# google-deepmind/mujoco_mpc

Measured on NVIDIA H100. Metric: env-steps/sec, higher is better.
Workload: dtype f32

## Files before the change

mujoco_mpc_b200/csrc/dev_data.cuh:

```cuda
#pragma once
#include <cuda_runtime.h>

#include "dev_model.h"

#ifndef MJPC_NO_COMPACT
#define MJPC_COMPACT 1
#endif
#ifdef MJPC_COMPACT
#define MJPC_ROLL _Pragma("unroll 1")
#define MJPC_HESS_ROLLED 1
#else
#define MJPC_ROLL
#endif

namespace mjpc_dev {

constexpr int kMaxSplinePoints = 64;
#define MJPC_D_ARRAYS(X)                                                                                          \
  X(qpos, M.nq) X(qvel, M.nv) X(ctrl, M.nu) X(qacc, M.nv) X(qacc_warmstart, M.nv) X(mocap_pos, 3 * M.nmocap)      \
  X(mocap_quat, 4 * M.nmocap) X(xpos, 3 * M.nbody) X(xquat, 4 * M.nbody) X(xmat, 9 * M.nbody)                     \
  X(xipos, 3 * M.nbody) X(ximat, 9 * M.nbody) X(xanchor, 3 * M.njnt) X(xaxis, 3 * M.njnt)                         \
  X(geom_xpos, 3 * M.ngeom) X(geom_xmat, 9 * M.ngeom) X(site_xpos, 3 * M.nsite) X(subtree_com, 3 * M.nbody)       \
  X(cinert, 10 * M.nbody) X(crb, 10 * M.nbody) X(cdof, 6 * M.nv) X(cdof_dot, 6 * M.nv) X(cvel, 6 * M.nbody)       \
  X(cacc, 6 * M.nbody) X(cfrc, 6 * M.nbody) X(cfrc_sub, 6 * M.nbody) X(subtree_linvel, 3 * M.nbody)               \
// ... 61 lines not shown
  const float* gkey;
  int xfrc_on;
  int npseudo;
  int warn;
  float time;
  unsigned* sync;
  int sync_slot;
  int sync_mode;
#ifdef MJPC_PHASE_TIMING
  long long tph[8], tlast;
#endif
};
#ifdef MJPC_PHASE_TIMING
#define PHASE(c, i) do { const long long t_ = clock64(); (c).tph[i] += t_ - (c).tlast; (c).tlast = t_; } while (0)
#else
#define PHASE(c, i) do { } while (0)
#endif
template <int V> struct IntC { static constexpr int v = V; };
constexpr int kHdrWords = (int)((sizeof(DevModel) + 15) / 16) * 4;
constexpr int kLayWords = (int)((sizeof(DevLayout) + 15) / 16) * 4;

struct DynSpec {
  static constexpr bool kStatic = false;
  static constexpr int kNV = 0, kNHPair = 0;
  static constexpr int kWide = 1, kTask = 0;
  static __device__ __forceinline__ const DevModel& hdr(const Ctx& c) { return *reinterpret_cast<const DevModel*>(g_smem + c.hdr); }
  static __device__ __forceinline__ const DevModel& model(const Ctx& c) { return hdr(c); }
  template <int ID> static __device__ __forceinline__ float* mf(const Ctx& c) { return g_smem + hdr(c).fo[ID]; }
  template <int ID> static __device__ __forceinline__ int* mi(const Ctx& c) {
    return reinterpret_cast<int*>(g_smem + c.ibase) + hdr(c).io[ID];
  }
  template <int ID> static __device__ __forceinline__ float* df(const Ctx& c) {
    return g_smem + c.dbase + reinterpret_cast<const DevLayout*>(g_smem + c.lay)->off[ID];
  }
};

template <class K, int W = 1, int T = 0>
struct StaticSpec {
  static constexpr bool kStatic = true;
  static constexpr int kWide = W, kTask = T;
  static __host__ __device__ constexpr int w(size_t byte_off, int i = 0) { return K::kModelWords[byte_off / 4 + i]; }
  struct View {
#define X(n) static constexpr int n = w(offsetof(DevModel, n));
    MJPC_M_INTS(X)
#undef X
  };
  static constexpr int kNV = View::nv, kNHPair = View::nhpair;
  static constexpr int kHdr = View::nf + View::ni;
  static constexpr int kData0 = kHdr + kHdrWords + kLayWords;
  static __device__ __forceinline__ const DevModel& hdr(const Ctx&) { return *reinterpret_cast<const DevModel*>(g_smem + kHdr); }
  static __device__ __forceinline__ View model(const Ctx&) { return View{}; }
  template <int ID> static __device__ __forceinline__ float* mf(const Ctx&) {
    return g_smem + IntC<w(offsetof(DevModel, fo), ID)>::v;
  }
  template <int ID> static __device__ __forceinline__ int* mi(const Ctx&) {
    return reinterpret_cast<int*>(g_smem) + IntC<View::nf + w(offsetof(DevModel, io), ID)>::v;
  }
  template <int ID> static __device__ __forceinline__ float* df(const Ctx&) {
    return g_smem + IntC<kData0 + K::kLayoutOff[ID]>::v;
  }
};

#define CM(c) (SP::hdr(c))
#define MF(n) (SP::template mf<F_##n>(c))
#define MI(n) (SP::template mi<I_##n>(c))
#define DF(n) (SP::template df<D_##n>(c))
#define DI(n) (reinterpret_cast<int*>(SP::template df<D_##n>(c)))

enum { WIDE_EXIT = 0, WIDE_HESSIAN = 1 };
struct WideBox { int cmd, ncon, nlim, ndrow, nefc; int task_exit, task_warn; float task_cost; };
// ... 274 lines not shown
  for (int i = N - 1; i >= 0; i--) {
    const float xi = __shfl_sync(kFull, y, i) * inv[i];
    const float lji = A[i * N + li];
    y = (lane == i) ? xi : (lane < i ? y - lji * xi : y);
  }
  if (lane < N) x[lane] = y;
  __syncwarp();
}

template <int NS>
__device__ __noinline__ void warp_chol_factor_solve(float* A, float* inv, float* x, const float* b, int n, int lane) {
#ifdef MJPC_CHOL_ROLLED2
  if constexpr (NS > 0 && NS <= 32) { warp_chol_factor_solve_rolled<NS>(A, inv, x, b, lane); return; }
  if (n == 18) { warp_chol_factor_solve_rolled<18>(A, inv, x, b, lane); return; }
#endif
#ifndef MJPC_CHOL_ROLLED
  if constexpr (NS > 0 && NS <= 32) { warp_chol_factor_solve_reg<NS>(A, x, b, lane); return; }
  if (n == 18) { warp_chol_factor_solve_reg<18>(A, x, b, lane); return; }
  if (n == 2) { warp_chol_factor_solve_reg<2>(A, x, b, lane); return; }
#endif
  warp_chol(A, inv, n, lane);
  warp_chol_solve(x, A, inv, b, n, lane);
}
#endif

}
```

mujoco_mpc_b200/csrc/dev_model.h:

```cpp
#pragma once
#include <cstdint>
#include <cstring>
#include <stdexcept>
#include <string>
#include <vector>

namespace mjpc_dev {

#define MJPC_F_ARRAYS(X)                                                                                         \
  X(body_pos) X(body_quat) X(body_ipos) X(body_iquat) X(body_mass) X(body_inertia) X(body_subtreemass)           \
  X(body_invweight0) X(jnt_pos) X(jnt_axis) X(jnt_range) X(jnt_stiffness) X(jnt_margin) X(jnt_solref)            \
  X(jnt_solimp) X(qpos0) X(qpos_spring) X(dof_damping) X(dof_armature) X(dof_frictionloss) X(dof_solref)         \
  X(dof_solimp) X(dof_invweight0) X(geom_size) X(geom_pos) X(geom_quat) X(geom_friction) X(geom_solmix)          \
  X(geom_solref) X(geom_solimp) X(geom_margin) X(geom_gap) X(geom_rbound) X(site_pos) X(site_quat)               \
  X(actuator_gear) X(actuator_gainprm) X(actuator_biasprm) X(actuator_ctrlrange) X(actuator_forcerange)          \
  X(key_qpos) X(task_weight) X(task_norm_parameter) X(task_parameters) X(task_state) X(wrap_coef) X(tendon_range)     \
  X(tendon_margin) X(tendon_solref) X(tendon_solimp) X(tendon_invweight0)
#define MJPC_I_ARRAYS(X)                                                                                         \
  X(body_parentid) X(body_rootid) X(body_jntnum) X(body_jntadr) X(body_dofnum) X(body_dofadr) X(body_mocapid)    \
  X(jnt_type) X(jnt_qposadr) X(jnt_dofadr) X(jnt_bodyid) X(jnt_limited) X(dof_bodyid) X(dof_jntid)               \
  X(dof_parentid) X(geom_type) X(geom_bodyid) X(geom_condim) X(geom_priority) X(site_bodyid) X(actuator_trnid) X(actuator_trntype)  \
  X(actuator_biastype) X(actuator_ctrllimited) X(actuator_forcelimited) X(pair_geom1) X(pair_geom2)              \
  X(ray_geoms) X(task_dim_norm_residual) X(task_norm) X(task_num_norm_parameter) X(task_trace_objtype)           \
  X(task_trace_objid) X(task_ids) X(tendon_adr) X(tendon_num) X(tendon_limited) X(wrap_dof) X(wrap_qposadr)
// ... 7 lines not shown
#undef X
      F_COUNT
};
enum IntArrayId {
#define X(n) I_##n,
  MJPC_I_ARRAYS(X) MJPC_I_DERIVED(X)
#undef X
      I_COUNT
};

enum { GEOM_PLANE = 0, GEOM_HFIELD, GEOM_SPHERE, GEOM_CAPSULE, GEOM_ELLIPSOID, GEOM_CYLINDER, GEOM_BOX };
enum { JNT_FREE = 0, JNT_BALL, JNT_SLIDE, JNT_HINGE };
enum { OBJ_BODY = 0, OBJ_XBODY, OBJ_GEOM, OBJ_SITE };
enum { CONE_PYRAMIDAL = 0, CONE_ELLIPTIC = 1 };
enum { RESIDUAL_PARTICLE = 0, RESIDUAL_PARTICLE_COPY = 1, RESIDUAL_CARTPOLE = 2, RESIDUAL_QUADRUPED_FLAT = 3,
       RESIDUAL_HUMANOID_STAND = 4, RESIDUAL_HUMANOID_TRACK = 5, RESIDUAL_SHADOW_REORIENT = 6 };

#define MJPC_M_INTS(X)                                                                                           \
  X(nq) X(nv) X(nu) X(nbody) X(njnt) X(ngeom) X(nsite) X(nmocap) X(nkey) X(npair) X(nray) X(nlevel) X(nmpair)    \
  X(ntendon)                                                                                                     \
  X(nfloss) X(nlimit) X(nhpair) X(cone) X(iterations) X(ls_iterations) X(disable_contact) X(disable_eulerdamp)  \
  X(disable_frictionloss) X(disable_limit) X(disable_refsafe) X(disable_warmstart) X(maxcon) X(maxefc)           \
  X(residual_id) X(num_residual) X(num_term) X(num_trace) X(num_parameters) X(task_state_size) X(any_damping)    \
  X(nf) X(ni)

struct DevModel {
#define X(n) int n;
  MJPC_M_INTS(X)
#undef X
  float timestep, impratio, tolerance, ls_tolerance, meaninertia, risk;
  float differentiable;
  float gravity[3];
  int fo[F_COUNT];
  int io[I_COUNT];
};

struct Blob {
  const uint8_t* p;
  size_t n;
  int nent;
  Blob(const void* data, size_t nbytes) : p((const uint8_t*)data), n(nbytes), nent(0) {
    if (!data || nbytes < 16 || std::memcmp(p, "MJPCB200", 8) != 0) throw std::runtime_error("bad model blob magic");
    std::memcpy(&nent, p + 12, 4);
    if ((size_t)16 + 56 * (size_t)nent > nbytes) throw std::runtime_error("truncated model blob");
  }
  bool find(const char* name, int* dt, int* cnt, int64_t* off) const {
    for (int i = 0; i < nent; i++) {
      const uint8_t* e = p + 16 + 56 * (size_t)i;
      if (std::strncmp((const char*)e, name, 40) == 0) {
        std::memcpy(dt, e + 40, 4); std::memcpy(cnt, e + 44, 4); std::memcpy(off, e + 48, 8);
        if ((size_t)*off + (size_t)*cnt * (*dt ? 8 : 4) > n) throw std::runtime_error("blob entry out of range");
        return true;
      }
    }
// ... 73 lines not shown
  }
  level_adr.push_back((int)level_body.size());
  M.nlevel = maxdepth;
  std::vector<int> subend(nb), lastdof(nb, -1), mlo(nb, 0), mhi(nb, 0);
  for (int bb = 0; bb < nb; bb++) {
    int e = bb + 1;
    while (e < nb && depth[e] > depth[bb]) e++;
    subend[bb] = e;
  }
  for (int bb = 1; bb < nb; bb++) {
    lastdof[bb] = dofnum[bb] > 0 ? dofadr[bb] + dofnum[bb] - 1 : lastdof[parent[bb]];
    uint64_t mask = 0;
    for (int d = lastdof[bb]; d >= 0; d = dofpar[d]) mask |= (uint64_t)1 << d;
    mlo[bb] = (int)(uint32_t)(mask & 0xffffffffu); mhi[bb] = (int)(uint32_t)(mask >> 32);
  }
  std::vector<int> mpi, mpj, fl, lj;
  for (int d = 0; d < nv; d++)
    for (int a = d; a >= 0; a = dofpar[a]) { mpi.push_back(d); mpj.push_back(a); }
  if (!M.disable_frictionloss)
    for (int d = 0; d < nv; d++) if (floss[d] > 0) fl.push_back(d);
  if (!M.disable_limit)
    for (int j = 0; j < M.njnt; j++) if (jlim[j] && (jtype[j] == JNT_SLIDE || jtype[j] == JNT_HINGE)) lj.push_back(j);
  M.nmpair = (int)mpi.size(); M.nfloss = (int)fl.size(); M.nlimit = (int)lj.size();
  M.any_damping = 0;
  for (double x : damping) if (x > 0) M.any_damping = 1;
  auto put = [&](int id, const std::vector<int>& v) { M.io[id] = (int)P.i.size(); P.i.insert(P.i.end(), v.begin(), v.end()); };
  put(I_level_adr, level_adr); put(I_level_body, level_body); put(I_body_subtreeend, subend);
  put(I_body_lastdof, lastdof); put(I_body_dofmask_lo, mlo); put(I_body_dofmask_hi, mhi);
  put(I_mpair_i, mpi); put(I_mpair_j, mpj); put(I_floss_dof, fl); put(I_limit_jnt, lj);
  {
    std::vector<uint8_t> pat((size_t)nv * nv, 0);
    for (size_t k = 0; k < mpi.size(); k++) pat[(size_t)mpi[k] * nv + mpj[k]] = 1;
    auto g1 = b.ints("pair_geom1"), g2 = b.ints("pair_geom2"), gb = b.ints("geom_bodyid");
    auto chain = [&](int bb) { uint64_t m = ((uint64_t)(uint32_t)mhi[bb] << 32) | (uint32_t)mlo[bb]; return m; };
    for (size_t k = 0; k < g1.size(); k++) {
      const uint64_t m1 = chain(gb[g1[k]]), m2 = chain(gb[g2[k]]);
      if (!m1 || !m2) continue;
      const uint64_t mm = m1 | m2;
      for (int r = 0; r < nv; r++) if ((mm >> r) & 1) for (int c2 = 0; c2 <= r; c2++) if ((mm >> c2) & 1) pat[(size_t)r * nv + c2] = 1;
    }
    {
      auto tadr = b.ints("tendon_adr"), tnum = b.ints("tendon_num"), wdof = b.ints("wrap_dof");
      for (size_t t = 0; t < tadr.size(); t++) {
        if (tnum[t] > 16) throw std::runtime_error("a tendon wraps more than 16 dofs (compact Jacobian width)");
        for (int a = tadr[t]; a < tadr[t] + tnum[t]; a++)
          for (int c2 = tadr[t]; c2 < tadr[t] + tnum[t]; c2++) {
// ... 36 lines not shown
```

mujoco_mpc_b200/csrc/dev_physics.cuh:

```cuda
#pragma once
#include "dev_data.cuh"

namespace mjpc_dev {



template <class SP>
__device__ __noinline__ void k_kinematics(Ctx& c) {
  auto&& M = SP::model(c);
  const int lane = c.lane;
  float *xpos = DF(xpos), *xquat = DF(xquat), *xmat = DF(xmat), *xipos = DF(xipos), *ximat = DF(ximat);
  float *xanchor = DF(xanchor), *xaxis = DF(xaxis);
  const float* qpos = DF(qpos);
  if (lane < 3) { xpos[lane] = 0; xipos[lane] = 0; }
  if (lane < 4) xquat[lane] = lane == 0 ? 1.f : 0.f;
  if (lane < 9) { float v = (lane % 4 == 0) ? 1.f : 0.f; xmat[lane] = v; ximat[lane] = v; }
  __syncwarp();
  const int *level_adr = MI(level_adr), *level_body = MI(level_body), *parentid = MI(body_parentid),
            *mocapid = MI(body_mocapid), *jntadr = MI(body_jntadr), *jntnum = MI(body_jntnum),
            *jtype = MI(jnt_type), *jqadr = MI(jnt_qposadr);
  const float *bpos = MF(body_pos), *bquat = MF(body_quat), *bipos = MF(body_ipos), *biquat = MF(body_iquat),
              *jpos = MF(jnt_pos), *jaxis = MF(jnt_axis), *qpos0 = MF(qpos0);
  for (int l = 0; l < M.nlevel; l++) {
    const int a = level_adr[l], e = level_adr[l + 1];
// ... 1014 lines not shown
  }
  __syncwarp();
  float* smooth = DF(qfrc_smooth);
  for (int i = lane; i < nv; i += 32) smooth[i] = passive[i] - bias[i] + qact[i];
  if (c.xfrc_on) {
    const float *xf = DF(xfrc), *cdof = DF(cdof), *xipos = DF(xipos), *scom = DF(subtree_com);
    const int *dbody = MI(dof_bodyid), *subend = MI(body_subtreeend), *rootid = MI(body_rootid);
    for (int i = lane; i < nv; i += 32) {
      const int b0 = dbody[i];
      const float* cd = cdof + 6 * i;
      float a = 0.f;
      MJPC_ROLL
      for (int b = b0; b < subend[b0]; b++) {
        float off[3], t[3];
        for (int q = 0; q < 3; q++) off[q] = xipos[3 * b + q] - scom[3 * rootid[b] + q];
        cross3(t, cd, off);
        const float* f = xf + 6 * b;
        for (int q = 0; q < 3; q++) a += (cd[3 + q] + t[q]) * f[q] + cd[q] * f[3 + q];
      }
      smooth[i] += a;
    }
  }
  __syncwarp();
  warp_chol_factor_solve<SP::kNV>(DF(qLD), DF(ldinv), DF(qacc_smooth), smooth, nv, lane);
}

template <class SP>
__device__ __noinline__ void k_reference(Ctx& c) {
  const int lane = c.lane;
  const float *qvel = DF(qvel), *K = DF(efc_K), *B = DF(efc_B), *imp = DF(efc_imp), *pos = DF(efc_pos),
              *margin = DF(efc_margin);
  float* aref = DF(efc_aref);
  const int nsimple = SP::model(c).nfloss + c.nlim;
  for (int i = lane; i < c.nefc; i += 32) {
    const float v = row_dot<SP>(c, i, nsimple, qvel);
    aref[i] = -B[i] * v - K[i] * imp[i] * (pos[i] - margin[i]);
  }
  __syncwarp();
}

template <class SP>
__device__ __noinline__ float k_update_constraint(Ctx& c, bool hess) {
  auto&& M = SP::model(c);
  const int lane = c.lane, nv = M.nv;
  const float *jar = DF(efc_jar), *D = DF(efc_D), *R = DF(efc_R), *floss = DF(efc_floss), *J = DF(efc_J);
  float *force = DF(efc_force), *X = DF(efc_W), *hw = DF(efc_hw), *xw = DF(efc_hc);
  int *state = DI(efc_state);
// ... 768 lines not shown
      const int i = min(b0 + lane, nv - 1);
      const bool on = b0 + lane < nv;
      const float a = Ma[i] - smooth[i] - qfc[i];
      if (on) grad[i] = a;
      g2 += on ? a * a : 0.f;
      const float m = fabsf(Ma[i]) + fabsf(smooth[i]) + fabsf(qfc[i]);
      ga += on ? m * m : 0.f;
    }
    const float gnorm2 = warp_sum(g2), gabs2 = warp_sum(ga);
    __syncwarp();
    if (iter > 0) {
      const float improvement = (old - cost) / scale_inv, gradient = sqrtf(gnorm2) / scale_inv;
      const float gfloor = kGradFloor * 1.1920929e-7f * sqrtf(gabs2) / scale_inv;
      if (gradient < fmaxf(tol, gfloor)) break;
      const bool resolvable = fabsf(old - cost) > 16.f * 1.1920929e-7f * fabsf(cost);
      if (resolvable) { if (improvement < tol) break; stalls = 0; }
      else if (gradient > 0.5f * prev_gradient && (alpha > 0.5f || ++stalls >= 3)) break;
      prev_gradient = gradient;
    }
    if (iter == M.iterations) break;
    PHASE(c, 4);
    k_hessian<SP>(c);
    PHASE(c, 5);
    warp_chol_factor_solve<SP::kNV>(DF(qH), DF(hinv), search, grad, nv, lane);
    PHASE(c, 6);
    for (int b0 = 0; b0 < nv; b0 += 32) { const int i = min(b0 + lane, nv - 1); const float v = -search[i]; __syncwarp(); if (b0 + lane < nv) search[i] = v; }
    __syncwarp();
    float q1 = 0, q2 = 0, sn = 0;
    for (int b0 = 0; b0 < nv; b0 += 32) {
      const int i = min(b0 + lane, nv - 1);
      const bool on = b0 + lane < nv;
      const float a = m_row_dot<SP>(qM, i, search, nv);
      if (on) Mv[i] = a;
      const float si = on ? search[i] : 0.f;
      q1 += si * (Ma[i] - smooth[i]);
      q2 += 0.5f * si * a;
      sn += si * si;
    }
    for (int b0 = 0; b0 < ne; b0 += 32) {
      const int i = min(b0 + lane, ne - 1);
      const float v = j_row_dot<SP>(c, i, nsimple, search, nv);
      if (b0 + lane < ne) Jv[i] = v;
    }
    q1 = warp_sum(q1); q2 = warp_sum(q2); sn = sqrtf(warp_sum(sn));
    __syncwarp();
    alpha = k_line_search<SP>(c, gauss, q1, q2, sn, scale_inv);
    if (alpha == 0.f) break;
// ... 29 lines not shown
  k_reference<SP>(c);
  PHASE(c, 3);
  k_solve<SP>(c);
  PHASE(c, 4);
}

template <class SP>
__device__ __noinline__ void k_euler(Ctx& c) {
  auto&& M = SP::model(c);
  const int lane = c.lane, nv = M.nv;
  const float h = CM(c).timestep;
  float *qacc = DF(qacc), *qvel = DF(qvel), *qpos = DF(qpos), *vt = DF(vtmp);
  const float* acc = qacc;
  if (M.any_damping && !M.disable_eulerdamp) {
    float *H = DF(qH), *qM = DF(qM), *smooth = DF(qfrc_smooth), *qfc = DF(qfrc_constraint);
    const float* damping = MF(dof_damping);
    MJPC_ROLL
    for (int w = lane; w < nv * nv; w += 32) {
      const int r = w / nv, s = w - r * nv;
      H[w] = qM[w] + (r == s ? h * damping[r] : 0.f);
    }
    for (int i = lane; i < nv; i += 32) vt[i] = smooth[i] + qfc[i];
    __syncwarp();
    warp_chol_factor_solve<SP::kNV>(H, DF(hinv), vt, vt, nv, lane);
    acc = vt;
  }
  for (int i = lane; i < nv; i += 32) qvel[i] += h * acc[i];
  __syncwarp();
  const int *jtype = MI(jnt_type), *jqadr = MI(jnt_qposadr), *jdadr = MI(jnt_dofadr);
  for (int j = lane; j < M.njnt; j += 32) {
    const int qa = jqadr[j], da = jdadr[j];
    const int t = jtype[j];
    if (t == JNT_FREE) {
      for (int q = 0; q < 3; q++) qpos[qa + q] += h * qvel[da + q];
      quat_integrate(qpos + qa + 3, qvel + da + 3, h);
    } else if (t == JNT_BALL) {
      quat_integrate(qpos + qa, qvel + da, h);
    } else {
      qpos[qa] += h * qvel[da];
    }
  }
  c.time += h;
  __syncwarp();
}

}
```

mujoco_mpc_b200/csrc/engine.cu:

```cuda
#include <cuda_runtime.h>
#include <dlfcn.h>
#include <nccl.h>

#include <algorithm>
#include <cmath>
#include <cstdio>
#include <cstdlib>
#include <cstring>
#include <string>
#include <vector>

#include "../../include/mjpc_b200.h"
#include "ilqg_kernels.cuh"
#include "rollout_kernels.cuh"

using namespace mjpc_dev;

namespace {
thread_local std::string g_last_error;
int fail(int code, const std::string& msg) { g_last_error = msg; return code; }

#define CUDA_TRY(expr)                                                                                     \
  do {                                                                                                     \
    cudaError_t e_ = (expr);                                                                               \
// ... 81 lines not shown
int set_smem(const void* fn, size_t bytes) {
  CUDA_TRY(mjpc_dev::raise_smem_limit(fn, bytes));
  return 0;
}

struct Staged { size_t state, mocap, tstate, end; };
Staged stage_common(mjpc_b200* h, const float* state, double time, const float* mocap) {
  const DevModel& M = h->pack.M;
  Staged s;
  size_t o = 0;
  s.state = o; std::memcpy(h->h_in + o, state, (M.nq + M.nv) * 4); o += M.nq + M.nv;
  s.mocap = o; if (M.nmocap) std::memcpy(h->h_in + o, mocap, 7 * M.nmocap * 4); o += 7 * M.nmocap;
  s.tstate = o;
  for (int i = 0; i < M.task_state_size; i++) {
    double v = h->task_state[i];
    if (std::find(h->time_idx.begin(), h->time_idx.end(), i) != h->time_idx.end()) v -= time;
    h->h_in[o + i] = (float)v;
  }
  o += M.task_state_size;
  s.end = o;
  return s;
}

int launch_rollout(mjpc_b200* h, const RolloutArgs& A_in) {
  RolloutArgs A = A_in;
  const int wpc = h->warps_per_cta;
  const size_t smem = h->smem_bytes(A.P, wpc);
  const int grid = (A.N + wpc - 1) / wpc;
  CUDA_TRY(cudaEventRecord(h->ev0, h->stream));
  const char* ns = std::getenv("MJPC_B200_NO_STATIC");
  const bool use_static = h->static_spec != 0 && wpc == 1 && !(ns && ns[0] == '1');
  {
    const char* ps = std::getenv("MJPC_B200_PAIR_SYNC");
    const bool on = !(ps && ps[0] == '0') && A.N > h->num_sms && A.N <= 2 * h->num_sms;
    A.pair_sync = on ? h->d_pair_sync : nullptr;
    A.pair_sync_mode = (ps && ps[0] >= '1' && ps[0] <= '9') ? std::atoi(ps) : 1;
    if (on) CUDA_TRY(cudaMemsetAsync(h->d_pair_sync, 0, (size_t)256 * 32 * sizeof(unsigned), h->stream));
  }
  const char* sh = std::getenv("MJPC_B200_SHAPE");
  const bool plain = sh && sh[0] == 'p' && sh[1] == 'l';
  if (use_static && h->static_spec == 1) {
    if (plain) rollout_kernel_quadruped_plain<<<grid, 32, smem, h->stream>>>(A);
    else rollout_kernel_quadruped<<<grid, kRolloutThreads, smem, h->stream>>>(A);
  } else if (use_static && h->static_spec == 2) {
    if (plain) rollout_kernel_humanoid_track_plain<<<grid, 32, smem, h->stream>>>(A);
    else rollout_kernel_humanoid_track<<<grid, kRolloutThreads, smem, h->stream>>>(A);
  } else {
    rollout_kernel<<<grid, 32 * wpc, smem, h->stream>>>(A);
// ... 544 lines not shown
  float* d = nullptr;
  CUDA_TRY(dalloc(&d, words));
  struct Guard { float* p; ~Guard() { cudaFree(p); } } guard{d};
  float *d_qpos = d, *d_qvel = d_qpos + B * nq, *d_ctrl = d_qvel + B * nv, *d_warm = d_ctrl + B * nu, *d_time = d_warm + B * nv,
        *d_qacc = d_time + B, *d_nq = d_qacc + B * nv, *d_nv = d_nq + B * nq, *d_res = d_nv + B * nv, *d_cost = d_res + B * nr,
        *d_counts = d_cost + B, *d_mocap = d_counts + 4 * (size_t)B, *d_ts = d_mocap + nm;
  std::vector<float> trel(B), ts(nts);
  for (int i = 0; i < B; i++) trel[i] = (float)(times[i] - time0);
  for (size_t i = 0; i < nts; i++) {
    double v = h->task_state[i];
    if (std::find(h->time_idx.begin(), h->time_idx.end(), (int)i) != h->time_idx.end()) v -= time0;
    ts[i] = (float)v;
  }
  CUDA_TRY(cudaMemcpy(d_qpos, qpos, B * nq * 4, cudaMemcpyHostToDevice));
  CUDA_TRY(cudaMemcpy(d_qvel, qvel, B * nv * 4, cudaMemcpyHostToDevice));
  CUDA_TRY(cudaMemcpy(d_ctrl, ctrl, B * nu * 4, cudaMemcpyHostToDevice));
  if (warmstart) CUDA_TRY(cudaMemcpy(d_warm, warmstart, B * nv * 4, cudaMemcpyHostToDevice));
  CUDA_TRY(cudaMemcpy(d_time, trel.data(), (size_t)B * 4, cudaMemcpyHostToDevice));
  if (nm) CUDA_TRY(cudaMemcpy(d_mocap, mocap, nm * 4, cudaMemcpyHostToDevice));
  if (nts) CUDA_TRY(cudaMemcpy(d_ts, ts.data(), nts * 4, cudaMemcpyHostToDevice));
  StepBatchArgs A;
  std::memset(&A, 0, sizeof(A));
  A.M = h->pack.M; A.L = make_layout(h->pack.M, 1); A.pack = h->d_pack;
  A.qpos = d_qpos; A.qvel = d_qvel; A.ctrl = d_ctrl; A.warmstart = warmstart ? d_warm : nullptr; A.mocap = d_mocap;
  A.task_state = nts ? d_ts : nullptr; A.time = d_time; A.B = B;
  A.qacc = d_qacc; A.next_qpos = d_nq; A.next_qvel = d_nv; A.residual = d_res; A.cost = d_cost; A.counts = (int*)d_counts;
  const size_t smem = h->smem_bytes(1, 1);
  const char* ns = std::getenv("MJPC_B200_NO_STATIC");
  const bool use_static = h->static_spec != 0 && !(ns && ns[0] == '1');
  const void* fn = use_static ? (h->static_spec == 1 ? (const void*)step_batch_kernel_quadruped : (const void*)step_batch_kernel_humanoid_track)
                              : (const void*)step_batch_kernel;
  if (int rc = set_smem(fn, smem)) return rc;
  CUDA_TRY(cudaEventRecord(h->ev0, h->stream));
  if (use_static && h->static_spec == 1) step_batch_kernel_quadruped<<<B, 32, smem, h->stream>>>(A);
  else if (use_static) step_batch_kernel_humanoid_track<<<B, 32, smem, h->stream>>>(A);
  else step_batch_kernel<<<B, 32, smem, h->stream>>>(A);
  CUDA_TRY(cudaEventRecord(h->ev1, h->stream));
  CUDA_TRY(cudaGetLastError());
  h->launches += 1;
  h->last_static = use_static ? 1 : 0;
  CUDA_TRY(cudaStreamSynchronize(h->stream));
  if (cudaEventElapsedTime(&h->last_ms, h->ev0, h->ev1) != cudaSuccess) cudaGetLastError();
  if (qacc) CUDA_TRY(cudaMemcpy(qacc, d_qacc, B * nv * 4, cudaMemcpyDeviceToHost));
  if (next_qpos) CUDA_TRY(cudaMemcpy(next_qpos, d_nq, B * nq * 4, cudaMemcpyDeviceToHost));
  if (next_qvel) CUDA_TRY(cudaMemcpy(next_qvel, d_nv, B * nv * 4, cudaMemcpyDeviceToHost));
  if (residual) CUDA_TRY(cudaMemcpy(residual, d_res, B * (size_t)M.num_residual * 4, cudaMemcpyDeviceToHost));
// ... 98 lines not shown
```

mujoco_mpc_b200/csrc/spec_humanoid_track.h:

```cpp
#pragma once
namespace mjpc_dev {
struct SpecHumanoidTrack {
  static constexpr int kNumModelWords = 153;
  static constexpr int kNumLayout = 101;
  static constexpr int kModelWords[512] = {
      28, 27, 21, 37, 22, 20, 38, 16, 1889, 159, 20, 7, 243, 2, 0, 21,
      378, 0, 100, 50, 0, 0, 0, 0, 0, 0, 32, 96, 5, 141, 21, 1,
      0, 2, 1, 2604, 2900, 1000593162, 1065353216, 841731191, 1008981770, 1087545275, 0, 0, 0, 0, -1055066685, 0,
      112, 260, 372, 520, 560, 672, 712, 788, 856, 924, 968, 992, 1016, 1060, 1172, 1200,
      1228, 1256, 1284, 1312, 1368, 1504, 1532, 1592, 1652, 1732, 1792, 1812, 1852, 1952, 1972, 1992,
      2012, 2128, 2280, 2304, 2368, 2432, 2476, 2520, 2520, 2544, 2568, 2568, 2572, 2576, 2580, 2584,
      2588, 2600, 0, 37, 74, 111, 148, 185, 222, 259, 281, 303, 325, 347, 369, 396,
      423, 450, 470, 490, 510, 530, 568, 589, 610, 631, 652, 673, 832, 991, 1011, 1032,
      1053, 1074, 1075, 1076, 1108, 1110, 1112, 1114, 1118, 1122, 1130, 1166, 1203, 1240, 1277, 1314,
      1557, 1800, 1800, 1821, 2199, 2577, 2604, 2641, 2678, 0, 0, 0, 0, 0, 0, 0,
      0, 0, 0, 0, 0, 0, 0, 0, 0, 0, 0, 0, 0, 0, 0, 0,
      0, 0, 0, 0, 0, 0, 0, 0, 0, 0, 0, 0, 0, 0, 0, 0,
      0, 0, 0, 0, 0, 0, 0, 0, 0, 0, 0, 0, 0, 0, 0, 0,
      0, 0, 0, 0, 0, 0, 0, 0, 0, 0, 0, 0, 0, 0, 0, 0,
      0, 0, 0, 0, 0, 0, 0, 0, 0, 0, 0, 0, 0, 0, 0, 0,
      0, 0, 0, 0, 0, 0, 0, 0, 0, 0, 0, 0, 0, 0, 0, 0,
      0, 0, 0, 0, 0, 0, 0, 0, 0, 0, 0, 0, 0, 0, 0, 0,
      0, 0, 0, 0, 0, 0, 0, 0, 0, 0, 0, 0, 0, 0, 0, 0,
      0, 0, 0, 0, 0, 0, 0, 0, 0, 0, 0, 0, 0, 0, 0, 0,
      0, 0, 0, 0, 0, 0, 0, 0, 0, 0, 0, 0, 0, 0, 0, 0,
      0, 0, 0, 0, 0, 0, 0, 0, 0, 0, 0, 0, 0, 0, 0, 0,
      0, 0, 0, 0, 0, 0, 0, 0, 0, 0, 0, 0, 0, 0, 0, 0,
      0, 0, 0, 0, 0, 0, 0, 0, 0, 0, 0, 0, 0, 0, 0, 0,
      0, 0, 0, 0, 0, 0, 0, 0, 0, 0, 0, 0, 0, 0, 0, 0,
      0, 0, 0, 0, 0, 0, 0, 0, 0, 0, 0, 0, 0, 0, 0, 0,
      0, 0, 0, 0, 0, 0, 0, 0, 0, 0, 0, 0, 0, 0, 0, 0,
      0, 0, 0, 0, 0, 0, 0, 0, 0, 0, 0, 0, 0, 0, 0, 0,
      0, 0, 0, 0, 0, 0, 0, 0, 0, 0, 0, 0, 0, 0, 0, 0,
      0, 0, 0, 0, 0, 0, 0, 0, 0, 0, 0, 0, 0, 0, 0, 0,
      0, 0, 0, 0, 0, 0, 0, 0, 0, 0, 0, 0, 0, 0, 0, 0,
      0, 0, 0, 0, 0, 0, 0, 0, 0, 0, 0, 0, 0, 0, 0, 0,
      0, 0, 0, 0, 0, 0, 0, 0, 0, 0, 0, 0, 0, 0, 0, 0,
  };
  static constexpr int kLayoutOff[256] = {
      0, 28, 56, 80, 108, 136, 184, 248, 360, 508, 844, 956, 1292, 1360, 1428, 1488,
      1668, 1784, 1896, 2268, 2640, 2804, 2968, 3192, 3416, 3640, 3864, 3976, 4088, 4820, 5552, 6284,
      6448, 6476, 6504, 6532, 6560, 6588, 6616, 6644, 6672, 6696, 6724, 6752, 6780, 6808, 6836, 6868,
      6964, 7252, 7412, 7476, 7636, 7668, 7700, 7732, 7764, 7796, 7828, 9364, 10388, 10420, 10932, 11796,
      11832, 12344, 13368, 13464, 13560, 16472, 18264, 18360, 18456, 18552, 18648, 18744, 18840, 18936, 19032, 19128,
      19224, 19320, 19416, 19512, 19608, 19704, 19800, 19896, 19992, 21144, 21176, 21208, 21784, 21816, 21848, 21944,
      22088, 22144, 22200, 22424, 22488, 0, 0, 0, 0, 0, 0, 0, 0, 0, 0, 0,
      0, 0, 0, 0, 0, 0, 0, 0, 0, 0, 0, 0, 0, 0, 0, 0,
      0, 0, 0, 0, 0, 0, 0, 0, 0, 0, 0, 0, 0, 0, 0, 0,
      0, 0, 0, 0, 0, 0, 0, 0, 0, 0, 0, 0, 0, 0, 0, 0,
      0, 0, 0, 0, 0, 0, 0, 0, 0, 0, 0, 0, 0, 0, 0, 0,
      0, 0, 0, 0, 0, 0, 0, 0, 0, 0, 0, 0, 0, 0, 0, 0,
      0, 0, 0, 0, 0, 0, 0, 0, 0, 0, 0, 0, 0, 0, 0, 0,
      0, 0, 0, 0, 0, 0, 0, 0, 0, 0, 0, 0, 0, 0, 0, 0,
      0, 0, 0, 0, 0, 0, 0, 0, 0, 0, 0, 0, 0, 0, 0, 0,
      0, 0, 0, 0, 0, 0, 0, 0, 0, 0, 0, 0, 0, 0, 0, 0,
  };
};
}
```

mujoco_mpc_b200/csrc/spec_quadruped.h:

```cpp
#pragma once
namespace mjpc_dev {
struct SpecQuadruped {
  static constexpr int kNumModelWords = 153;
  static constexpr int kNumLayout = 101;
  static constexpr int kModelWords[512] = {
      19, 18, 12, 16, 13, 42, 6, 2, 2, 395, 4, 4, 117, 0, 12, 12,
      171, 1, 100, 50, 0, 0, 0, 0, 0, 0, 32, 96, 3, 42, 9, 1,
      11, 31, 1, 2124, 2144, 1008981770, 1092616192, 841731191, 1008981770, 1074405708, 0, 0, 0, 0, -1055066685, 0,
      48, 112, 160, 224, 240, 288, 304, 336, 376, 416, 444, 460, 476, 504, 572, 592,
      612, 632, 652, 672, 708, 800, 820, 948, 1076, 1244, 1372, 1416, 1500, 1712, 1756, 1800,
      1844, 1864, 1888, 1900, 1936, 1972, 1996, 2020, 2060, 2072, 2080, 2092, 2124, 2124, 2124, 2124,
      2124, 2124, 0, 16, 32, 48, 64, 80, 96, 112, 125, 138, 151, 164, 177, 195,
      213, 231, 273, 315, 357, 399, 405, 417, 429, 441, 453, 465, 860, 1255, 1259, 1268,
      1277, 1286, 1287, 1288, 1305, 1305, 1305, 1305, 1305, 1305, 1310, 1325, 1341, 1357, 1373, 1389,
      1506, 1623, 1635, 1647, 1818, 1989, 2007, 2023, 2039, 0, 0, 0, 0, 0, 0, 0,
      0, 0, 0, 0, 0, 0, 0, 0, 0, 0, 0, 0, 0, 0, 0, 0,
      0, 0, 0, 0, 0, 0, 0, 0, 0, 0, 0, 0, 0, 0, 0, 0,
      0, 0, 0, 0, 0, 0, 0, 0, 0, 0, 0, 0, 0, 0, 0, 0,
      0, 0, 0, 0, 0, 0, 0, 0, 0, 0, 0, 0, 0, 0, 0, 0,
      0, 0, 0, 0, 0, 0, 0, 0, 0, 0, 0, 0, 0, 0, 0, 0,
      0, 0, 0, 0, 0, 0, 0, 0, 0, 0, 0, 0, 0, 0, 0, 0,
      0, 0, 0, 0, 0, 0, 0, 0, 0, 0, 0, 0, 0, 0, 0, 0,
      0, 0, 0, 0, 0, 0, 0, 0, 0, 0, 0, 0, 0, 0, 0, 0,
      0, 0, 0, 0, 0, 0, 0, 0, 0, 0, 0, 0, 0, 0, 0, 0,
      0, 0, 0, 0, 0, 0, 0, 0, 0, 0, 0, 0, 0, 0, 0, 0,
      0, 0, 0, 0, 0, 0, 0, 0, 0, 0, 0, 0, 0, 0, 0, 0,
      0, 0, 0, 0, 0, 0, 0, 0, 0, 0, 0, 0, 0, 0, 0, 0,
      0, 0, 0, 0, 0, 0, 0, 0, 0, 0, 0, 0, 0, 0, 0, 0,
      0, 0, 0, 0, 0, 0, 0, 0, 0, 0, 0, 0, 0, 0, 0, 0,
      0, 0, 0, 0, 0, 0, 0, 0, 0, 0, 0, 0, 0, 0, 0, 0,
      0, 0, 0, 0, 0, 0, 0, 0, 0, 0, 0, 0, 0, 0, 0, 0,
      0, 0, 0, 0, 0, 0, 0, 0, 0, 0, 0, 0, 0, 0, 0, 0,
      0, 0, 0, 0, 0, 0, 0, 0, 0, 0, 0, 0, 0, 0, 0, 0,
      0, 0, 0, 0, 0, 0, 0, 0, 0, 0, 0, 0, 0, 0, 0, 0,
      0, 0, 0, 0, 0, 0, 0, 0, 0, 0, 0, 0, 0, 0, 0, 0,
      0, 0, 0, 0, 0, 0, 0, 0, 0, 0, 0, 0, 0, 0, 0, 0,
      0, 0, 0, 0, 0, 0, 0, 0, 0, 0, 0, 0, 0, 0, 0, 0,
  };
  static constexpr int kLayoutOff[256] = {
      0, 20, 40, 52, 72, 92, 100, 108, 156, 220, 364, 412, 556, 596, 636, 764,
      1144, 1164, 1212, 1372, 1532, 1640, 1748, 1844, 1940, 2036, 2132, 2180, 2228, 2552, 2876, 3200,
      3308, 3328, 3348, 3368, 3388, 3408, 3428, 3448, 3468, 3480, 3500, 3520, 3540, 3560, 3580, 3612,
      3708, 3996, 4156, 4220, 4380, 4412, 4444, 4476, 4508, 4540, 4572, 6108, 7132, 7164, 7676, 8252,
      8288, 8800, 9824, 9920, 10016, 12096, 13376, 13472, 13568, 13664, 13760, 13856, 13952, 14048, 14144, 14240,
      14336, 14432, 14528, 14624, 14720, 14816, 14912, 15008, 15104, 16256, 16288, 16320, 16896, 16928, 16960, 17056,
      17100, 17140, 17176, 17272, 17336, 0, 0, 0, 0, 0, 0, 0, 0, 0, 0, 0,
      0, 0, 0, 0, 0, 0, 0, 0, 0, 0, 0, 0, 0, 0, 0, 0,
      0, 0, 0, 0, 0, 0, 0, 0, 0, 0, 0, 0, 0, 0, 0, 0,
      0, 0, 0, 0, 0, 0, 0, 0, 0, 0, 0, 0, 0, 0, 0, 0,
      0, 0, 0, 0, 0, 0, 0, 0, 0, 0, 0, 0, 0, 0, 0, 0,
      0, 0, 0, 0, 0, 0, 0, 0, 0, 0, 0, 0, 0, 0, 0, 0,
      0, 0, 0, 0, 0, 0, 0, 0, 0, 0, 0, 0, 0, 0, 0, 0,
      0, 0, 0, 0, 0, 0, 0, 0, 0, 0, 0, 0, 0, 0, 0, 0,
      0, 0, 0, 0, 0, 0, 0, 0, 0, 0, 0, 0, 0, 0, 0, 0,
      0, 0, 0, 0, 0, 0, 0, 0, 0, 0, 0, 0, 0, 0, 0, 0,
  };
};
}
```

mujoco_mpc_b200/gen_spec.py:

```python
from __future__ import annotations

import ctypes as C
import os

import numpy as np

HERE = os.path.dirname(os.path.abspath(__file__))
SPECS = {"quadruped": "SpecQuadruped", "humanoid_track": "SpecHumanoidTrack"}
PAD_MODEL, PAD_LAYOUT = 512, 256


def header_text(struct: str, name: str, words) -> str:
    nm, nl = int(words[0]), int(words[1])
    model, layout = list(words[2:2 + nm]), list(words[2 + nm:2 + nm + nl])
    assert nm <= PAD_MODEL and nl <= PAD_LAYOUT
    model += [0] * (PAD_MODEL - nm)
    layout += [0] * (PAD_LAYOUT - nl)

    def rows(v):
        return "\n".join("      " + ", ".join(str(int(x)) for x in v[i:i + 16]) + "," for i in range(0, len(v), 16))

    return (f"// GENERATED by mujoco_mpc_b200/gen_spec.py from models.load(\"{name}\") - do not edit.\n"
            f"// DevModel header words and per-trajectory state offsets of the task model (see dev_data.cuh: StaticSpec).\n"
            f"#pragma once\nnamespace mjpc_dev {{\nstruct {struct} {{\n"
            f"  static constexpr int kNumModelWords = {nm};\n  static constexpr int kNumLayout = {nl};\n"
            f"  static constexpr int kModelWords[{PAD_MODEL}] = {{\n{rows(model)}\n  }};\n"
            f"  static constexpr int kLayoutOff[{PAD_LAYOUT}] = {{\n{rows(layout)}\n  }};\n}};\n}}  // namespace mjpc_dev\n")


def spec_words(lib, blob: bytes):
    from .engine import ModelBlob
    buf = C.create_string_buffer(blob, len(blob))
    mb = ModelBlob(C.cast(buf, C.c_void_p), len(blob))
    out = np.zeros(2 + PAD_MODEL + PAD_LAYOUT, np.int32)
    n = lib.mjpc_b200_spec_words(C.byref(mb), out.ctypes.data_as(C.POINTER(C.c_int)), len(out))
    if n < 0:
        raise RuntimeError("mjpc_b200_spec_words failed: %d" % n)
    return out[:n]


def generate(so_path: str | None = None) -> bool:
    from . import models
    from .blob import to_blob
    from .build import SO
    lib = C.CDLL(so_path or SO)
    changed = False
    for name, struct in SPECS.items():
        text = header_text(struct, name, spec_words(lib, to_blob(models.load(name))))
        path = os.path.join(HERE, "csrc", f"spec_{name}.h")
        old = open(path).read() if os.path.exists(path) else ""
        if old != text:
            open(path, "w").write(text)
            changed = True
    return changed


if __name__ == "__main__":
    print("spec tables", "updated" if generate() else "up to date")
```

Measured before the change: 2.532 million.

## Add sparse tree LDL^T solve using compile-time dof parent tables

Replaces the dense warp Cholesky factor/solve with a sparsity-aware LDL^T factorization. It follows the kinematic dof tree, which is baked into the static spec headers as kDofParent and is used for models with at most 24 dofs. Elimination only touches ancestor entries, so it skips fill work that the tree structure makes zero. In the Newton solver it is used only when there are no dense constraint rows. An environment variable can force the old dense path, and a model hash field plus an A/B profiling script are added. The risk is that numerics differ slightly from dense Cholesky and the unrolled code grows.

```diff
diff --git a/mujoco_mpc_b200/csrc/dev_data.cuh b/mujoco_mpc_b200/csrc/dev_data.cuh
--- a/mujoco_mpc_b200/csrc/dev_data.cuh
+++ b/mujoco_mpc_b200/csrc/dev_data.cuh
@@ -107,6 +107,8 @@
 
 struct DynSpec {
   static constexpr bool kStatic = false;
+  static constexpr bool kTree = false;
+  using Tables = void;
   static constexpr int kNV = 0, kNHPair = 0;
   static constexpr int kWide = 1, kTask = 0;
   static __device__ __forceinline__ const DevModel& hdr(const Ctx& c) { return *reinterpret_cast<const DevModel*>(g_smem + c.hdr); }
@@ -131,6 +133,8 @@
 #undef X
   };
   static constexpr int kNV = View::nv, kNHPair = View::nhpair;
+  static constexpr bool kTree = kNV > 0 && kNV <= 24;
+  using Tables = K;
   static constexpr int kHdr = View::nf + View::ni;
   static constexpr int kData0 = kHdr + kHdrWords + kLayWords;
   static __device__ __forceinline__ const DevModel& hdr(const Ctx&) { return *reinterpret_cast<const DevModel*>(g_smem + kHdr); }
@@ -451,6 +455,72 @@
   warp_chol(A, inv, n, lane);
   warp_chol_solve(x, A, inv, b, n, lane);
 }
-#endif
-
-}
+
+template <int N>
+struct DofTree {
+  int h[N];
+  unsigned anc[N];
+  unsigned desc[N];
+  int maxh;
+};
+template <int N>
+__host__ __device__ constexpr DofTree<N> make_dof_tree(const int* par) {
+  DofTree<N> t{};
+  for (int k = N - 1; k >= 0; k--)
+    if (par[k] >= 0 && t.h[par[k]] < t.h[k] + 1) t.h[par[k]] = t.h[k] + 1;
+  for (int k = 0; k < N; k++) {
+    if (t.h[k] > t.maxh) t.maxh = t.h[k];
+    for (int a = par[k]; a >= 0; a = par[a]) { t.anc[k] |= 1u << a; t.desc[a] |= 1u << k; }
+  }
+  return t;
+}
+template <class K, int N>
+__device__ __noinline__ void warp_tree_ldl_solve(const float* A, float* x, const float* b, int lane) {
+  static_assert(N > 0 && N <= 32, "one dof per lane");
+  constexpr DofTree<N> T = make_dof_tree<N>(K::kDofParent);
+  float row[N], il[N];
+  const int li = lane < N ? lane : N - 1;
+#pragma unroll
+  for (int k = 0; k < N; k++) row[k] = A[li * N + k];
+  float y = b[li];
+  __syncwarp();
+#pragma unroll
+  for (int l = 0; l <= T.maxh; l++) {
+#pragma unroll
+    for (int k = 0; k < N; k++) {
+      if (T.h[k] != l) continue;
+      float p = __shfl_sync(kFull, row[k], k);
+      if (p < kMinVal) p = kMinVal;
+      il[k] = 1.0f / p;
+      const float yk = __shfl_sync(kFull, y, k) * il[k];
+      const float m = mask_pick(row[k], (T.anc[k] >> lane) & 1u, 0.f, false);
+      y -= m * yk;
+#pragma unroll
+      for (int a = 0; a < N; a++)
+        if ((T.anc[k] >> a) & 1u) row[a] -= m * (__shfl_sync(kFull, row[a], k) * il[k]);
+    }
+  }
+#pragma unroll
+  for (int l = T.maxh; l >= 0; l--) {
+#pragma unroll
+    for (int k = 0; k < N; k++) {
+      if (T.h[k] != l) continue;
+      const float xk = __shfl_sync(kFull, y, k) * il[k];
+      const float yd = y - mask_pick(row[k], (T.desc[k] >> lane) & 1u, 0.f, false) * xk;
+      y = mask_pick(xk, lane == k, yd, lane != k);
+    }
+  }
+  if (lane < N) x[lane] = y;
+  __syncwarp();
+}
+
+template <class SP>
+__device__ __forceinline__ void factor_solve(const Ctx& c, float* A, float* inv, float* x, const float* b, bool tree) {
+  if constexpr (SP::kTree) {
+    if (tree && CM(c).dense_factor == 0.f) { warp_tree_ldl_solve<typename SP::Tables, SP::kNV>(A, x, b, c.lane); return; }
+  }
+  warp_chol_factor_solve<SP::kNV>(A, inv, x, b, SP::model(c).nv, c.lane);
+}
+#endif
+
+}
diff --git a/mujoco_mpc_b200/csrc/dev_model.h b/mujoco_mpc_b200/csrc/dev_model.h
--- a/mujoco_mpc_b200/csrc/dev_model.h
+++ b/mujoco_mpc_b200/csrc/dev_model.h
@@ -53,7 +53,7 @@
   X(nfloss) X(nlimit) X(nhpair) X(cone) X(iterations) X(ls_iterations) X(disable_contact) X(disable_eulerdamp)  \
   X(disable_frictionloss) X(disable_limit) X(disable_refsafe) X(disable_warmstart) X(maxcon) X(maxefc)           \
   X(residual_id) X(num_residual) X(num_term) X(num_trace) X(num_parameters) X(task_state_size) X(any_damping)    \
-  X(nf) X(ni)
+  X(dof_tree) X(nf) X(ni)
 
 struct DevModel {
 #define X(n) int n;
@@ -61,6 +61,7 @@
 #undef X
   float timestep, impratio, tolerance, ls_tolerance, meaninertia, risk;
   float differentiable;
+  float dense_factor;
   float gravity[3];
   int fo[F_COUNT];
   int io[I_COUNT];
@@ -180,6 +181,11 @@
   if (!M.disable_limit)
     for (int j = 0; j < M.njnt; j++) if (jlim[j] && (jtype[j] == JNT_SLIDE || jtype[j] == JNT_HINGE)) lj.push_back(j);
   M.nmpair = (int)mpi.size(); M.nfloss = (int)fl.size(); M.nlimit = (int)lj.size();
+  {
+    uint32_t hsh = 2166136261u;
+    for (int d = 0; d < nv; d++) { hsh ^= (uint32_t)(dofpar[d] + 1); hsh *= 16777619u; }
+    M.dof_tree = (int)hsh;
+  }
   M.any_damping = 0;
   for (double x : damping) if (x > 0) M.any_damping = 1;
   auto put = [&](int id, const std::vector<int>& v) { M.io[id] = (int)P.i.size(); P.i.insert(P.i.end(), v.begin(), v.end()); };
diff --git a/mujoco_mpc_b200/csrc/dev_physics.cuh b/mujoco_mpc_b200/csrc/dev_physics.cuh
--- a/mujoco_mpc_b200/csrc/dev_physics.cuh
+++ b/mujoco_mpc_b200/csrc/dev_physics.cuh
@@ -1060,7 +1060,7 @@
     }
   }
   __syncwarp();
-  warp_chol_factor_solve<SP::kNV>(DF(qLD), DF(ldinv), DF(qacc_smooth), smooth, nv, lane);
+  factor_solve<SP>(c, DF(qLD), DF(ldinv), DF(qacc_smooth), smooth, true);
 }
 
 template <class SP>
@@ -1875,7 +1875,7 @@
     PHASE(c, 4);
     k_hessian<SP>(c);
     PHASE(c, 5);
-    warp_chol_factor_solve<SP::kNV>(DF(qH), DF(hinv), search, grad, nv, lane);
+    factor_solve<SP>(c, DF(qH), DF(hinv), search, grad, c.ndrow == 0);
     PHASE(c, 6);
     for (int b0 = 0; b0 < nv; b0 += 32) { const int i = min(b0 + lane, nv - 1); const float v = -search[i]; __syncwarp(); if (b0 + lane < nv) search[i] = v; }
     __syncwarp();
@@ -1951,7 +1951,7 @@
     }
     for (int i = lane; i < nv; i += 32) vt[i] = smooth[i] + qfc[i];
     __syncwarp();
-    warp_chol_factor_solve<SP::kNV>(H, DF(hinv), vt, vt, nv, lane);
+    factor_solve<SP>(c, H, DF(hinv), vt, vt, true);
     acc = vt;
   }
   for (int i = lane; i < nv; i += 32) qvel[i] += h * acc[i];
diff --git a/mujoco_mpc_b200/csrc/engine.cu b/mujoco_mpc_b200/csrc/engine.cu
--- a/mujoco_mpc_b200/csrc/engine.cu
+++ b/mujoco_mpc_b200/csrc/engine.cu
@@ -127,8 +127,14 @@
   return s;
 }
 
+float dense_factor_env() {
+  const char* f = std::getenv("MJPC_B200_FACTOR");
+  return f && f[0] == 'd' ? 1.f : 0.f;
+}
+
 int launch_rollout(mjpc_b200* h, const RolloutArgs& A_in) {
   RolloutArgs A = A_in;
+  A.M.dense_factor = dense_factor_env();
   const int wpc = h->warps_per_cta;
   const size_t smem = h->smem_bytes(A.P, wpc);
   const int grid = (A.N + wpc - 1) / wpc;
@@ -719,6 +725,7 @@
   StepBatchArgs A;
   std::memset(&A, 0, sizeof(A));
   A.M = h->pack.M; A.L = make_layout(h->pack.M, 1); A.pack = h->d_pack;
+  A.M.dense_factor = dense_factor_env();
   A.qpos = d_qpos; A.qvel = d_qvel; A.ctrl = d_ctrl; A.warmstart = warmstart ? d_warm : nullptr; A.mocap = d_mocap;
   A.task_state = nts ? d_ts : nullptr; A.time = d_time; A.B = B;
   A.qacc = d_qacc; A.next_qpos = d_nq; A.next_qvel = d_nv; A.residual = d_res; A.cost = d_cost; A.counts = (int*)d_counts;
diff --git a/mujoco_mpc_b200/csrc/spec_humanoid_track.h b/mujoco_mpc_b200/csrc/spec_humanoid_track.h
--- a/mujoco_mpc_b200/csrc/spec_humanoid_track.h
+++ b/mujoco_mpc_b200/csrc/spec_humanoid_track.h
@@ -1,19 +1,19 @@
 #pragma once
 namespace mjpc_dev {
 struct SpecHumanoidTrack {
-  static constexpr int kNumModelWords = 153;
+  static constexpr int kNumModelWords = 155;
   static constexpr int kNumLayout = 101;
   static constexpr int kModelWords[512] = {
       28, 27, 21, 37, 22, 20, 38, 16, 1889, 159, 20, 7, 243, 2, 0, 21,
       378, 0, 100, 50, 0, 0, 0, 0, 0, 0, 32, 96, 5, 141, 21, 1,
-      0, 2, 1, 2604, 2900, 1000593162, 1065353216, 841731191, 1008981770, 1087545275, 0, 0, 0, 0, -1055066685, 0,
-      112, 260, 372, 520, 560, 672, 712, 788, 856, 924, 968, 992, 1016, 1060, 1172, 1200,
-      1228, 1256, 1284, 1312, 1368, 1504, 1532, 1592, 1652, 1732, 1792, 1812, 1852, 1952, 1972, 1992,
-      2012, 2128, 2280, 2304, 2368, 2432, 2476, 2520, 2520, 2544, 2568, 2568, 2572, 2576, 2580, 2584,
-      2588, 2600, 0, 37, 74, 111, 148, 185, 222, 259, 281, 303, 325, 347, 369, 396,
-      423, 450, 470, 490, 510, 530, 568, 589, 610, 631, 652, 673, 832, 991, 1011, 1032,
-      1053, 1074, 1075, 1076, 1108, 1110, 1112, 1114, 1118, 1122, 1130, 1166, 1203, 1240, 1277, 1314,
-      1557, 1800, 1800, 1821, 2199, 2577, 2604, 2641, 2678, 0, 0, 0, 0, 0, 0, 0,
+      0, 2, 1, -440014593, 2604, 2900, 1000593162, 1065353216, 841731191, 1008981770, 1087545275, 0, 0, 0, 0, 0,
+      -1055066685, 0, 112, 260, 372, 520, 560, 672, 712, 788, 856, 924, 968, 992, 1016, 1060,
+      1172, 1200, 1228, 1256, 1284, 1312, 1368, 1504, 1532, 1592, 1652, 1732, 1792, 1812, 1852, 1952,
+      1972, 1992, 2012, 2128, 2280, 2304, 2368, 2432, 2476, 2520, 2520, 2544, 2568, 2568, 2572, 2576,
+      2580, 2584, 2588, 2600, 0, 37, 74, 111, 148, 185, 222, 259, 281, 303, 325, 347,
+      369, 396, 423, 450, 470, 490, 510, 530, 568, 589, 610, 631, 652, 673, 832, 991,
+      1011, 1032, 1053, 1074, 1075, 1076, 1108, 1110, 1112, 1114, 1118, 1122, 1130, 1166, 1203, 1240,
+      1277, 1314, 1557, 1800, 1800, 1821, 2199, 2577, 2604, 2641, 2678, 0, 0, 0, 0, 0,
       0, 0, 0, 0, 0, 0, 0, 0, 0, 0, 0, 0, 0, 0, 0, 0,
       0, 0, 0, 0, 0, 0, 0, 0, 0, 0, 0, 0, 0, 0, 0, 0,
       0, 0, 0, 0, 0, 0, 0, 0, 0, 0, 0, 0, 0, 0, 0, 0,
@@ -55,5 +55,11 @@
       0, 0, 0, 0, 0, 0, 0, 0, 0, 0, 0, 0, 0, 0, 0, 0,
       0, 0, 0, 0, 0, 0, 0, 0, 0, 0, 0, 0, 0, 0, 0, 0,
   };
+  static constexpr int kDofParent[64] = {
+      -1, 0, 1, 2, 3, 4, 5, 6, 7, 8, 9, 10, 11, 12, 13, 8,
+      15, 16, 17, 18, 19, 5, 21, 22, 5, 24, 25, -1, -1, -1, -1, -1,
+      -1, -1, -1, -1, -1, -1, -1, -1, -1, -1, -1, -1, -1, -1, -1, -1,
+      -1, -1, -1, -1, -1, -1, -1, -1, -1, -1, -1, -1, -1, -1, -1, -1,
+  };
 };
 }
diff --git a/mujoco_mpc_b200/csrc/spec_quadruped.h b/mujoco_mpc_b200/csrc/spec_quadruped.h
--- a/mujoco_mpc_b200/csrc/spec_quadruped.h
+++ b/mujoco_mpc_b200/csrc/spec_quadruped.h
@@ -1,19 +1,19 @@
 #pragma once
 namespace mjpc_dev {
 struct SpecQuadruped {
-  static constexpr int kNumModelWords = 153;
+  static constexpr int kNumModelWords = 155;
   static constexpr int kNumLayout = 101;
   static constexpr int kModelWords[512] = {
       19, 18, 12, 16, 13, 42, 6, 2, 2, 395, 4, 4, 117, 0, 12, 12,
       171, 1, 100, 50, 0, 0, 0, 0, 0, 0, 32, 96, 3, 42, 9, 1,
-      11, 31, 1, 2124, 2144, 1008981770, 1092616192, 841731191, 1008981770, 1074405708, 0, 0, 0, 0, -1055066685, 0,
-      48, 112, 160, 224, 240, 288, 304, 336, 376, 416, 444, 460, 476, 504, 572, 592,
-      612, 632, 652, 672, 708, 800, 820, 948, 1076, 1244, 1372, 1416, 1500, 1712, 1756, 1800,
-      1844, 1864, 1888, 1900, 1936, 1972, 1996, 2020, 2060, 2072, 2080, 2092, 2124, 2124, 2124, 2124,
-      2124, 2124, 0, 16, 32, 48, 64, 80, 96, 112, 125, 138, 151, 164, 177, 195,
-      213, 231, 273, 315, 357, 399, 405, 417, 429, 441, 453, 465, 860, 1255, 1259, 1268,
-      1277, 1286, 1287, 1288, 1305, 1305, 1305, 1305, 1305, 1305, 1310, 1325, 1341, 1357, 1373, 1389,
-      1506, 1623, 1635, 1647, 1818, 1989, 2007, 2023, 2039, 0, 0, 0, 0, 0, 0, 0,
+      11, 31, 1, 727244426, 2124, 2144, 1008981770, 1092616192, 841731191, 1008981770, 1074405708, 0, 0, 0, 0, 0,
+      -1055066685, 0, 48, 112, 160, 224, 240, 288, 304, 336, 376, 416, 444, 460, 476, 504,
+      572, 592, 612, 632, 652, 672, 708, 800, 820, 948, 1076, 1244, 1372, 1416, 1500, 1712,
+      1756, 1800, 1844, 1864, 1888, 1900, 1936, 1972, 1996, 2020, 2060, 2072, 2080, 2092, 2124, 2124,
+      2124, 2124, 2124, 2124, 0, 16, 32, 48, 64, 80, 96, 112, 125, 138, 151, 164,
+      177, 195, 213, 231, 273, 315, 357, 399, 405, 417, 429, 441, 453, 465, 860, 1255,
+      1259, 1268, 1277, 1286, 1287, 1288, 1305, 1305, 1305, 1305, 1305, 1305, 1310, 1325, 1341, 1357,
+      1373, 1389, 1506, 1623, 1635, 1647, 1818, 1989, 2007, 2023, 2039, 0, 0, 0, 0, 0,
       0, 0, 0, 0, 0, 0, 0, 0, 0, 0, 0, 0, 0, 0, 0, 0,
       0, 0, 0, 0, 0, 0, 0, 0, 0, 0, 0, 0, 0, 0, 0, 0,
       0, 0, 0, 0, 0, 0, 0, 0, 0, 0, 0, 0, 0, 0, 0, 0,
@@ -55,5 +55,11 @@
       0, 0, 0, 0, 0, 0, 0, 0, 0, 0, 0, 0, 0, 0, 0, 0,
       0, 0, 0, 0, 0, 0, 0, 0, 0, 0, 0, 0, 0, 0, 0, 0,
   };
+  static constexpr int kDofParent[64] = {
+      -1, 0, 1, 2, 3, 4, 5, 6, 7, 5, 9, 10, 5, 12, 13, 5,
+      15, 16, -1, -1, -1, -1, -1, -1, -1, -1, -1, -1, -1, -1, -1, -1,
+      -1, -1, -1, -1, -1, -1, -1, -1, -1, -1, -1, -1, -1, -1, -1, -1,
+      -1, -1, -1, -1, -1, -1, -1, -1, -1, -1, -1, -1, -1, -1, -1, -1,
+  };
 };
 }
diff --git a/mujoco_mpc_b200/gen_spec.py b/mujoco_mpc_b200/gen_spec.py
--- a/mujoco_mpc_b200/gen_spec.py
+++ b/mujoco_mpc_b200/gen_spec.py
@@ -10,12 +10,15 @@
 PAD_MODEL, PAD_LAYOUT = 512, 256
 
 
-def header_text(struct: str, name: str, words) -> str:
+def header_text(struct: str, name: str, words, dof_parent) -> str:
     nm, nl = int(words[0]), int(words[1])
     model, layout = list(words[2:2 + nm]), list(words[2 + nm:2 + nm + nl])
     assert nm <= PAD_MODEL and nl <= PAD_LAYOUT
     model += [0] * (PAD_MODEL - nm)
     layout += [0] * (PAD_LAYOUT - nl)
+    par = [int(x) for x in dof_parent]
+    assert len(par) <= 64
+    par += [-1] * (64 - len(par))
 
     def rows(v):
         return "\n".join("      " + ", ".join(str(int(x)) for x in v[i:i + 16]) + "," for i in range(0, len(v), 16))
@@ -25,7 +28,9 @@
             f"#pragma once\nnamespace mjpc_dev {{\nstruct {struct} {{\n"
             f"  static constexpr int kNumModelWords = {nm};\n  static constexpr int kNumLayout = {nl};\n"
             f"  static constexpr int kModelWords[{PAD_MODEL}] = {{\n{rows(model)}\n  }};\n"
-            f"  static constexpr int kLayoutOff[{PAD_LAYOUT}] = {{\n{rows(layout)}\n  }};\n}};\n}}  // namespace mjpc_dev\n")
+            f"  static constexpr int kLayoutOff[{PAD_LAYOUT}] = {{\n{rows(layout)}\n  }};\n"
+            f"  // dof_parentid: the compile-time kinematic tree of the tree LDL^T solve (dev_data.cuh: warp_tree_ldl_solve)\n"
+            f"  static constexpr int kDofParent[64] = {{\n{rows(par)}\n  }};\n}};\n}}  // namespace mjpc_dev\n")
 
 
 def spec_words(lib, blob: bytes):
@@ -46,7 +51,8 @@
     lib = C.CDLL(so_path or SO)
     changed = False
     for name, struct in SPECS.items():
-        text = header_text(struct, name, spec_words(lib, to_blob(models.load(name))))
+        m = models.load(name)
+        text = header_text(struct, name, spec_words(lib, to_blob(m)), m.dof_parentid)
         path = os.path.join(HERE, "csrc", f"spec_{name}.h")
         old = open(path).read() if os.path.exists(path) else ""
         if old != text:
diff --git a/profiles/ab_factor.py b/profiles/ab_factor.py
--- /dev/null
+++ b/profiles/ab_factor.py
@@ -0,0 +1,25 @@
+import os, sys, numpy as np
+R = os.path.dirname(os.path.dirname(os.path.abspath(__file__))); sys.path.insert(0, R); sys.path.insert(0, os.path.join(R, "tests"))
+from conftest import get_model
+from mujoco_mpc_b200.engine import Engine
+m = get_model("quadruped")
+N = int(sys.argv[1]) if len(sys.argv) > 1 else 256
+e = Engine(m, N, 64)
+d = np.load(os.path.join(R, "profiles", "inputs_quadruped_256x64.npz"))
+state, mocap, kt = d["state"], d["mocap"], d["kt"]
+kn = np.concatenate([d["knots"]] * ((N + 255) // 256))[:N]
+modes = ("dense", "tree")
+ms = {k: [] for k in modes}; ret = {}
+for rep in range(12):
+    for k in modes:
+        os.environ["MJPC_B200_FACTOR"] = k
+        r, _, _ = e.rollout_spline(state, 0.0, mocap, kn, kt, 2, 64)
+        ret[k] = r
+        if rep >= 2: ms[k].append(e.last_kernel_ms)
+for k, v in ms.items():
+    print("N=%d %s: kernel ms min %.3f median %.3f max %.3f" % (N, "dense Cholesky" if k == "dense" else "tree LDL^T   ", min(v), np.median(v), max(v)))
+print("tree LDL^T vs dense: %.1f %% less kernel time" % (100 * (1 - np.median(ms["tree"]) / np.median(ms["dense"]))))
+a, b = ret["tree"].astype(float), ret["dense"].astype(float)
+rel = np.abs(a - b) / np.abs(b)
+print("returns: median rel diff %.2e, max %.2e (candidate %d), > 1e-4: %d of %d; argmin tree %d dense %d" % (
+    np.median(rel), rel.max(), int(rel.argmax()), int((rel > 1e-4).sum()), N, int(a.argmin()), int(b.argmin())))
```

Result: no change. 2.540 million (median of 6 runs) (+0.3%).
